# videosegmentation/video_segment

Measured on AMD Instinct MI355X. Metric: over-segmented frames/sec at 1080p, higher is better.
Workload: dtype f32

## Files before the change

### include/vsg.h

```cpp
#ifndef VSG_H_
#define VSG_H_

#include <stddef.h>
#include <stdint.h>

#ifdef __cplusplus
extern "C" {
#endif

#define VSG_OK 0
#define VSG_ERR_INVALID -1
#define VSG_ERR_DEVICE -2
#define VSG_ERR_STATE -3
#define VSG_ERR_INTERNAL -4

#define VSG_MEM_HOST 0
#define VSG_MEM_DEVICE 1

typedef struct vsg_stream vsg_stream;
typedef struct vsg_graph vsg_graph;

typedef struct vsg_options {
  int presmoothing;
  float frac_min_region_size;
// ... 215 lines not shown
                          const int32_t** nbr_csr_ptr, const int32_t** nbr_csr_idx);
int vsg_graph_get_intervals(vsg_graph* g, int frame, const vsg_interval** intervals, size_t* n);
int vsg_graph_smoothed(vsg_graph* g, int t, float* out );
int vsg_graph_spatial_buckets(vsg_graph* g, int t, uint16_t* out );
int vsg_graph_temporal_buckets(vsg_graph* g, int t, uint16_t* out , int32_t* prev_idx);
int vsg_graph_list_slots(vsg_graph* g, int list, uint32_t* slots_out, int32_t* offsets_out);
int vsg_graph_node_roots(vsg_graph* g, int32_t* out);
int vsg_graph_node_states(vsg_graph* g, int32_t* root, float* mean, int32_t* size, int32_t* constraint,
                          uint8_t* flags);
int vsg_graph_merge_stats(const vsg_graph* g, int64_t* forced_regular_small);
int vsg_graph_timings(const vsg_graph* g, vsg_timings* t);
int vsg_graph_diagnostics(const vsg_graph* g, vsg_diagnostics* d);
int vsg_graph_merge_paths(const vsg_graph* g, vsg_merge_paths* out);
int vsg_graph_spine_paths(const vsg_graph* g, vsg_spine_paths* out);

int vsg_debug_sort_pairs(const uint32_t* keys, const uint32_t* values, int n, int end_bit,
                         uint32_t* keys_out, uint32_t* values_out, int device);
int vsg_debug_sort_pairs_timed(const uint32_t* keys, const uint32_t* values, int n, int end_bit,
                               uint32_t* keys_out, uint32_t* values_out, int device, int impl, int reps,
                               double* avg_us);
int vsg_debug_exclusive_sum(const int32_t* in, int n, int32_t* out, int64_t* total);
int vsg_debug_runs_of_sorted_keys(const uint32_t* keys, int n, int32_t* seg_off, int32_t* seg_cnt,
                                  int32_t* num_runs);

#ifdef __cplusplus
}
#endif
#endif
```

### video_segment_amd/_lib.py

```python
import ctypes as C
import os
import subprocess

_HERE = os.path.dirname(os.path.abspath(__file__))
CSRC_DIR = os.path.join(_HERE, "csrc")
LIB_PATH = os.path.join(_HERE, "lib", "libvsg_hip.so")

VSG_OK = 0
VSG_ERR_INVALID, VSG_ERR_DEVICE, VSG_ERR_STATE, VSG_ERR_INTERNAL = -1, -2, -3, -4
VSG_MEM_HOST = 0
VSG_MEM_DEVICE = 1


class VsgOptions(C.Structure):
    _fields_ = [
        ("presmoothing", C.c_int),
        ("frac_min_region_size", C.c_float),
        ("chunk_size", C.c_int),
        ("chunk_overlap_ratio", C.c_float),
        ("num_constraint_frames", C.c_int),
        ("enforce_n4_connectivity", C.c_int),
        ("enforce_spatial_connectedness", C.c_int),
        ("color_distance", C.c_int),
        ("device", C.c_int),
# ... 117 lines not shown
    "vsg_stream_create", "vsg_stream_destroy", "vsg_stream_process_frame", "vsg_stream_chunk_size",
    "vsg_stream_result_bytes", "vsg_stream_result_id_image", "vsg_stream_last_merge_stats",
    "vsg_stream_keep_node_states", "vsg_stream_last_node_states",
    "vsg_stream_last_timings", "vsg_stream_last_diagnostics", "vsg_stream_last_merge_paths", "vsg_stream_last_spine_paths",
    "vsg_stream_last_boundary_paths",
    "vsg_stream_last_smoothed", "vsg_stream_export_halo",
    "vsg_stream_import_halo", "vsg_stream_expect_halo", "vsg_stream_restart",
    "vsg_chain_create", "vsg_chain_destroy", "vsg_chain_info", "vsg_chain_send_halo",
    "vsg_chain_recv_halo", "vsg_chain_exchange_halo",
    "vsg_regionseg_default_options", "vsg_regionseg_create", "vsg_regionseg_destroy", "vsg_regionseg_process_frame",
    "vsg_regionseg_result_bytes", "vsg_bgr_to_lab",
    "vsg_graph_create", "vsg_graph_destroy", "vsg_graph_add_frame_bgr",
    "vsg_graph_add_frame_features", "vsg_graph_add_virtual_frame", "vsg_graph_add_temporal",
    "vsg_graph_add_frame_features_temporal", "vsg_graph_list_slots",
    "vsg_graph_finish_building", "vsg_graph_segment_spatially", "vsg_graph_segment", "vsg_graph_obtain_results",
    "vsg_graph_num_frames", "vsg_graph_num_regions", "vsg_graph_num_neighbor_links",
    "vsg_graph_region_sizes", "vsg_graph_index_image", "vsg_graph_get_regions",
    "vsg_graph_get_intervals", "vsg_graph_smoothed",
    "vsg_graph_spatial_buckets", "vsg_graph_temporal_buckets", "vsg_graph_node_roots",
    "vsg_graph_node_states",
    "vsg_graph_merge_stats", "vsg_graph_timings", "vsg_graph_diagnostics", "vsg_graph_merge_paths",
    "vsg_graph_spine_paths",
    "vsg_debug_sort_pairs", "vsg_debug_sort_pairs_timed", "vsg_debug_exclusive_sum", "vsg_debug_runs_of_sorted_keys",
]


def build(force=False):
    subprocess.check_call(["make", "-C", CSRC_DIR, "-j8", "-s"])
    return LIB_PATH


_lib = None


def lib():
    global _lib
    if _lib is not None:
        return _lib
    if not os.path.exists(LIB_PATH):
        raise RuntimeError(
            "libvsg_hip.so is missing (%s): build the HIP extension first; there is no fallback "
            "path" % LIB_PATH)
    try:
        import torch
    except ImportError:
        pass
# ... 55 lines not shown
    L.vsg_graph_segment.argtypes = [vp, C.c_int, C.c_int]
    L.vsg_graph_obtain_results.argtypes = [vp, C.c_int, C.c_int, C.c_int]
    L.vsg_graph_num_frames.argtypes = [vp]
    L.vsg_graph_num_regions.argtypes = [vp]
    L.vsg_graph_num_neighbor_links.argtypes = [vp]
    L.vsg_graph_num_neighbor_links.restype = C.c_int64
    L.vsg_graph_region_sizes.argtypes = [vp, vp, vp]
    L.vsg_graph_index_image.argtypes = [vp, C.c_int, vp]
    L.vsg_graph_get_regions.argtypes = [vp, C.POINTER(vp), C.POINTER(C.c_size_t), C.POINTER(vp),
                                        C.POINTER(vp)]
    L.vsg_graph_get_intervals.argtypes = [vp, C.c_int, C.POINTER(vp), C.POINTER(C.c_size_t)]
    L.vsg_graph_smoothed.argtypes = [vp, C.c_int, vp]
    L.vsg_graph_spatial_buckets.argtypes = [vp, C.c_int, vp]
    L.vsg_graph_temporal_buckets.argtypes = [vp, C.c_int, vp, vp]
    L.vsg_graph_node_roots.argtypes = [vp, vp]
    L.vsg_graph_node_states.argtypes = [vp, vp, vp, vp, vp, vp]
    L.vsg_graph_merge_stats.argtypes = [vp, vp]
    L.vsg_graph_timings.argtypes = [vp, C.POINTER(VsgTimings)]
    L.vsg_graph_diagnostics.argtypes = [vp, C.POINTER(VsgDiagnostics)]
    L.vsg_graph_merge_paths.argtypes = [vp, C.POINTER(VsgMergePaths)]
    L.vsg_graph_spine_paths.argtypes = [vp, C.POINTER(VsgSpinePaths)]
    L.vsg_debug_exclusive_sum.argtypes = [vp, C.c_int, vp, C.POINTER(C.c_int64)]
    L.vsg_debug_runs_of_sorted_keys.argtypes = [vp, C.c_int, vp, vp, C.POINTER(C.c_int32)]
    _lib = L
    return L


class VsgError(RuntimeError):

    def __init__(self, msg, code=None):
        super().__init__(msg)
        self.code = code


def memory_stats(device=-1):
    st = VsgMemoryStats()
    check(lib().vsg_device_memory_stats(device, C.byref(st)))
    return st.as_dict()


def memory_trim(device=-1):
    check(lib().vsg_device_memory_trim(device))


def memory_limit(nbytes, device=-1):
    check(lib().vsg_device_memory_limit(device, int(nbytes)))
# ... 6 lines not shown
```

### video_segment_amd/csrc/capi.cpp

```cpp
#include <algorithm>
#include <cstring>
#include <memory>
#include <string>
#include <vector>

#include <rccl/rccl.h>

#include <chrono>
#include <cstdio>
#include <fstream>
#include <thread>

#include "../../include/vsg.h"
#include "region_segmentation.h"
#include "scan_device.h"
#include "stream.h"

namespace {

thread_local std::string g_last_error;

template <class F>
int Guard(F&& f) {
  try {
// ... 759 lines not shown
}

int vsg_debug_runs_of_sorted_keys(const uint32_t* keys, int n, int32_t* seg_off, int32_t* seg_cnt,
                                  int32_t* num_runs) {
  return Guard([&] {
    VSG_REQUIRE(keys && seg_off && seg_cnt && num_runs && n >= 0, VSG_ERR_INVALID, "bad argument");
    RequireDevice(-1);
    if (n == 0) return;
    vsg::DevBuf<uint32_t> d_keys((size_t)n);
    vsg::DevBuf<int32_t> d_off((size_t)n), d_cnt((size_t)n), sums(vsg::kScanMaxTiles), d_runs(1);
    DebugStream st;
    VSG_HIP(hipMemcpyAsync(d_keys.get(), keys, (size_t)n * 4, hipMemcpyHostToDevice, st.s));
    VSG_HIP(hipMemcpyAsync(d_off.get(), seg_off, (size_t)n * 4, hipMemcpyHostToDevice, st.s));
    VSG_HIP(hipMemcpyAsync(d_cnt.get(), seg_cnt, (size_t)n * 4, hipMemcpyHostToDevice, st.s));
    vsg::RunsOfSortedKeys(vsg::ScanScratch{sums.get(), nullptr}, d_keys.get(), n, d_off.get(), d_cnt.get(), d_runs.get(),
                          st.s);
    VSG_HIP(hipMemcpyAsync(seg_off, d_off.get(), (size_t)n * 4, hipMemcpyDeviceToHost, st.s));
    VSG_HIP(hipMemcpyAsync(seg_cnt, d_cnt.get(), (size_t)n * 4, hipMemcpyDeviceToHost, st.s));
    VSG_HIP(hipMemcpyAsync(num_runs, d_runs.get(), 4, hipMemcpyDeviceToHost, st.s));
    VSG_HIP(hipStreamSynchronize(st.s));
  });
}

int vsg_graph_create(int width, int height, int max_frames, int l1, int device, vsg_graph** out) {
  return Guard([&] {
    VSG_REQUIRE(out, VSG_ERR_INVALID, "null argument");
    RequireFrameSize(width, height);
    RequireDevice(device);
    std::unique_ptr<vsg_graph> g(new vsg_graph);
    g->device = ResolveDevice(device);
    DeviceGuard dg(g->device);
    g->W = width;
    g->H = height;
    g->wh = (size_t)width * height;
    VSG_HIP(hipStreamCreateWithFlags(&g->stream, hipStreamNonBlocking));
    g->g.reset(new vsg::DenseGraphHip(width, height, max_frames, l1 != 0, g->stream));
    g->pre.reset(new vsg::Preprocessor(width, height, g->stream));
    std::memset(&g->timings, 0, sizeof(g->timings));
    *out = g.release();
  });
}

void vsg_graph_destroy(vsg_graph* g) {
  if (!g) return;
  (void)Guard([&] {
    DeviceGuard dg(g->device);
// ... 388 lines not shown
```

### video_segment_amd/csrc/device_graph.h

```cpp
#ifndef VSG_DEVICE_GRAPH_H_
#define VSG_DEVICE_GRAPH_H_

#include <functional>

#include "common.h"

namespace vsg {

constexpr uint8_t kFlagFinalized = 1;
constexpr uint8_t kFlagNoDesc = 2;
constexpr uint8_t kFlagTentative = 4;
constexpr uint8_t kFlagHub = 8;
constexpr uint8_t kFlagHubBroken = 16;
constexpr uint8_t kFlagHubExcluded = 32;
constexpr int kHubExclCap = 16384;
constexpr int kHubMaxAttempts = 4;
constexpr int kHubMaxSplits = 64;
constexpr int kHubCutCap = 64;
constexpr int kHubListInts = 4 + kHubExclCap + 3 * kHubCutCap;

struct NodeArrays {
  int32_t* parent;
  float4* desc_sz;
  int32_t* cons;
// ... 40 lines not shown
  int32_t* chunk;
  int32_t* offsets;
  uint32_t* slots;
  int per_px;
};
constexpr int kEdgeSortMaxLists = 2;
void LaunchSpatialKeys(const float* feat, int W, int H, int l1, uint16_t* keys, int32_t* hist,
                       hipStream_t s);
void LaunchTemporalKeys(const float* cur, const float* prev, const float* flow, int W, int H,
                        int l1, int is_virtual, uint16_t* keys, int32_t* prev_idx, int32_t* hist,
                        hipStream_t s);
void LaunchBucketSort(const EdgeSortList* lists, int n_lists, size_t n_px, hipStream_t s);
void LaunchInitNodes(const float* feat, size_t n, int base, const int32_t* cons_in,
                     NodeArrays nodes, hipStream_t s);
void LaunchInitVirtualNodes(const int32_t* labels, size_t n, int base, int num_labels,
                            int32_t* first_scratch, NodeArrays nodes, hipStream_t s);

constexpr int kScanMaxTiles = 4096;
struct ScanScratch {
  int32_t* sums;
  hipStream_t owner = nullptr;
};

void DebugExclusiveSum(const ScanScratch& sc, const int32_t* in, int32_t* out, int n, int32_t* total, hipStream_t s);

size_t SortPairsU32HandTempBytes(int n);
void SortPairsU32Hand(void* temp, size_t temp_bytes, const uint32_t* keys_in, uint32_t* keys_out,
                      const uint32_t* vals_in, uint32_t* vals_out, int n, int end_bit, hipStream_t s);
size_t SortPairsU32LibTempBytes(int n);
void SortPairsU32Lib(void* temp, size_t temp_bytes, const uint32_t* keys_in, uint32_t* keys_out,
                     const uint32_t* vals_in, uint32_t* vals_out, int n, int end_bit, hipStream_t s);
size_t SortPairsU32TempBytes(int n);
void SortPairsU32(void* temp, size_t temp_bytes, const uint32_t* keys_in, uint32_t* keys_out,
                  const uint32_t* vals_in, uint32_t* vals_out, int n, int end_bit, hipStream_t s);
bool SortPairsU32TakesHand(int n);
size_t SortKeysU64TempBytes(int n);
void SortKeysU64(void* temp, size_t temp_bytes, const unsigned long long* in,
                 unsigned long long* out, int n,
                 hipStream_t s);
size_t UniqueU64TempBytes(int n);
void UniqueU64(void* temp, size_t temp_bytes, const unsigned long long* in,
               unsigned long long* out,
               int32_t* num_out, int n, hipStream_t s);

constexpr int kMailValues = 4;
struct MailSlot {
// ... 259 lines not shown
```

### video_segment_amd/csrc/merge_spine.hip

```cpp
#include <algorithm>
#include <chrono>
#include <cstdlib>
#include <cstdio>
#include <unordered_map>
#include <vector>

#include "merge_common.h"
#include "scan_device.h"

namespace vsg {

namespace {

constexpr int kNone = -1;

static inline unsigned Blocks(size_t n) { return (unsigned)((n + 255) / 256); }

__device__ __forceinline__ int CompOf(const int32_t* __restrict__ comp_base, int K, int e) {
  int lo = 0, hi = K;
  while (hi - lo > 1) {
    const int mid = (lo + hi) >> 1;
    if (comp_base[mid] <= e) lo = mid; else hi = mid;
  }
  return lo;
}

// ... 11 lines not shown
    const int lo = CompOf(comp_base, K, e);
    const int pos = comp_off[lo] + (e - comp_base[lo]);
    u = s_ra[pos];
    v = s_rb[pos];
    eu[e] = u;
    ev[e] = v;
    estate[e] = 0;
  }
  const int pu = __shfl_up(u, 1), pv = __shfl_up(v, 1);
  const bool first = (threadIdx.x & 63) == 0;
  if (valid && (first || (u != pu && u != pv))) {
    cc[u] = u;
    best[u] = 0xffffffffu;
  }
  if (valid && v != u && (first || (v != pu && v != pv))) {
    cc[v] = v;
    best[v] = 0xffffffffu;
  }
}

constexpr int kAliveSlots = 32;
__device__ __forceinline__ uint32_t BorKey(int round, int e) { return ((uint32_t)(31 - round) << 27) | (uint32_t)e; }

__global__ __launch_bounds__(256) void k_bor_min(int n, const int32_t* __restrict__ list,
                                                  const int32_t* __restrict__ list_len, int round,
                                                  const int32_t* __restrict__ eu,
                                                  const int32_t* __restrict__ ev, int32_t* __restrict__ estate,
                                                  int32_t* __restrict__ cc, uint32_t* __restrict__ best,
                                                  int32_t* __restrict__ ecu, int32_t* __restrict__ ecv,
                                                  int32_t* __restrict__ alive, const int32_t* __restrict__ gate,
                                                  int32_t* __restrict__ next_len) {
  if (blockIdx.x == 0 && threadIdx.x == 0) *next_len = 0;
  if (gate && *gate == 0) return;
  const int i = blockIdx.x * 256 + threadIdx.x;
  if (list_len) n = min(n, *list_len);
  const int e = i < n ? (list ? list[i] : i) : -1;
  bool live = false;
  int cu = -1, cv = -1;
  if (e >= 0 && round == 0) {
    cu = eu[e];
    cv = ev[e];
    live = true;
  } else if (e >= 0 && estate[e] == 0) {
    cu = CcFind(cc, eu[e]);
    cv = CcFind(cc, ev[e]);
    if (cu == cv) {
      estate[e] = 2;
      cu = cv = -1;
    } else {
      live = true;
      ecu[e] = cu;
      ecv[e] = cv;
    }
  }
  const int pu = __shfl_up(cu, 1), pv = __shfl_up(cv, 1), pe = __shfl_up(e, 1);
  if (live) {
    const uint32_t key = BorKey(round, e);
    const bool has_prev = (threadIdx.x & 63) != 0 && pe < e;
    if (!(has_prev && (cu == pu || cu == pv)) && key < best[cu]) atomicMin(&best[cu], key);
    if (!(has_prev && (cv == pu || cv == pv)) && key < best[cv]) atomicMin(&best[cv], key);
  }
  const int cnt = __syncthreads_count(live);
  if (cnt && threadIdx.x == 0) atomicAdd(&alive[(blockIdx.x % kAliveSlots) * 16], cnt);
}

__global__ __launch_bounds__(256) void k_bor_hook(int n, const int32_t* __restrict__ list,
                                                   const int32_t* __restrict__ list_len, int round,
                                                   const int32_t* __restrict__ eu, const int32_t* __restrict__ ev,
                                                   int32_t* __restrict__ estate, int32_t* __restrict__ cc,
                                                   const uint32_t* __restrict__ best,
                                                   const int32_t* __restrict__ ecu, const int32_t* __restrict__ ecv,
                                                   const int32_t* __restrict__ alive,
                                                   unsigned long long* __restrict__ mail, unsigned mail_seq,
                                                   const int32_t* __restrict__ gate, int32_t* __restrict__ total_out) {
  const int i = blockIdx.x * 256 + threadIdx.x;
  const bool idle = gate && *gate == 0;
  if (blockIdx.x == 0) {
    int v = (!idle && threadIdx.x < kAliveSlots) ? alive[threadIdx.x * 16] : 0;
    for (int off = 32; off > 0; off >>= 1) v += __shfl_down(v, off);
    if (threadIdx.x == 0) {
      *total_out = v;
      MailPost(mail, mail_seq, 0, v);
    }
  }
  if (idle) return;
  if (list_len) n = min(n, *list_len);
  if (i >= n) return;
  const int e = list ? list[i] : i;
  if (estate[e] != 0) return;
  const uint32_t key = BorKey(round, e);
  const int cu = round == 0 ? eu[e] : ecu[e], cv = round == 0 ? ev[e] : ecv[e];
  if (best[cu] == key || best[cv] == key) {
    CcUnion(cc, eu[e], ev[e]);
    estate[e] = 1;
  }
}

constexpr int kBorCompactPer = 8;
__global__ __launch_bounds__(256) void k_bor_compact(int n, const int32_t* __restrict__ list,
                                                      const int32_t* __restrict__ list_len,
                                                      const int32_t* __restrict__ estate, int32_t* __restrict__ out,
                                                      int32_t* __restrict__ out_len) {
  __shared__ int wave_tot[4];
  __shared__ int block_base;
  if (list_len) n = min(n, *list_len);
  const int lane = threadIdx.x & 63, w = threadIdx.x >> 6;
  int e[kBorCompactPer];
  unsigned long long m[kBorCompactPer];
  int mine = 0;
#pragma unroll
  for (int k = 0; k < kBorCompactPer; ++k) {
    const int i = (blockIdx.x * kBorCompactPer + k) * 256 + threadIdx.x;
    e[k] = i < n ? (list ? list[i] : i) : -1;
    const bool keep = e[k] >= 0 && estate[e[k]] == 0;
    m[k] = __ballot(keep);
    mine += (int)__popcll(m[k]);
  }
  if (lane == 0) wave_tot[w] = mine;
  __syncthreads();
  if (threadIdx.x == 0) {
    const int total = wave_tot[0] + wave_tot[1] + wave_tot[2] + wave_tot[3];
    block_base = total ? atomicAdd(out_len, total) : 0;
  }
  __syncthreads();
  int at = block_base;
  for (int q = 0; q < w; ++q) at += wave_tot[q];
#pragma unroll
  for (int k = 0; k < kBorCompactPer; ++k) {
    if ((m[k] >> lane) & 1ull) out[at + (int)__popcll(m[k] & ((1ull << lane) - 1ull))] = e[k];
    at += (int)__popcll(m[k]);
  }
}

constexpr int kRootStride = 16;
__global__ __launch_bounds__(256) void k_spine_pick_root(int mE, int K, const int32_t* __restrict__ eu,
                                                          const int32_t* __restrict__ ev,
                                                          const int32_t* __restrict__ comp_base, NodeArrays nodes,
                                                          unsigned long long* __restrict__ root_key) {
  __shared__ unsigned long long red[256];
  __shared__ int comp0;
  const int i = blockIdx.x * 256 + threadIdx.x;
  const int e = i < K ? comp_base[i] : (i - K) * kRootStride;
  unsigned long long key = 0;
  int k = -1;
  if (e < mE) {
    k = CompOf(comp_base, K, e);
    const int u = eu[e], v = ev[e];
    const unsigned su = (unsigned)__float_as_int(nodes.desc_sz[u].w);
    const unsigned sv = (unsigned)__float_as_int(nodes.desc_sz[v].w);
    const unsigned long long ku = ((unsigned long long)su << 32) | (unsigned)(~u);
    const unsigned long long kv = ((unsigned long long)sv << 32) | (unsigned)(~v);
    key = ku > kv ? ku : kv;
  }
// ... 951 lines not shown
    out[2 * i] = seg_off[seg];
    out[2 * i + 1] = cnt;
  }
}

struct Pool {
  int32_t* base;
  size_t cap, used = 0;
  bool ok = true;
  size_t mark() const { return used; }
  void release(size_t m) { used = m; }
  int32_t* take(size_t n) {
    n = (n + 63) & ~(size_t)63;
    if (used + n > cap) {
      ok = false;
      return base;
    }
    int32_t* p = base + used;
    used += n;
    return p;
  }
};

}

size_t SpinePoolInts(size_t max_edges) { return 16 * max_edges + 64 * 1024; }

int SelectLargeSegments(int max_segs, const int32_t* num_segs, const int32_t* seg_off, const int32_t* seg_cnt,
                        int min_cnt, long long max_edges, MergeScratch& S, hipStream_t s, SpineInput* out,
                        long long* wanted_edges) {
  out->segs.clear();
  if (wanted_edges) *wanted_edges = 0;
  Mailbox& mb = *S.mail;
  VSG_REQUIRE(mb.list_cap >= 2 * kSpineListCap, -4, "mailbox list too small");
  std::vector<int32_t> large(1 + 2 * kSpineListCap);
  int found = 0;
  for (;; min_cnt *= 4) {
    int32_t* d_found = TakeZeroed(S, 1);
    hipLaunchKernelGGL(k_list_large_segments, dim3(Blocks(max_segs)), dim3(256), 0, s, max_segs, num_segs, seg_off,
                       seg_cnt, min_cnt, d_found, mb.list_dev);
    const MailSlot m = NextMail(mb);
    LaunchMailPost(m, d_found, nullptr, nullptr, nullptr, s);
    MailWait(m, 1, &found, s);
    if (found <= kSpineListCap) break;
  }
  large[0] = found;
// ... 16 lines not shown
    all += sizes[(size_t)i];
  }
  if (wanted_edges) *wanted_edges = all;
  std::sort(sizes.begin(), sizes.end(), std::greater<int>());
  long long sum = 0;
  int taken = 0, thr = 0x7fffffff;
  for (int i = 0; i < found && i < 256;) {
    int j = i;
    long long group = 0;
    while (j < found && sizes[(size_t)j] == sizes[(size_t)i]) group += sizes[(size_t)j++];
    if (sum + group > max_edges || j > 256) break;
    sum += group;
    taken = j;
    thr = sizes[(size_t)i];
    i = j;
  }
  if (taken == 0) return 0x7fffffff;
  for (int i = 0; i < found; ++i) {
    if (large[2 + 2 * i] >= thr) out->segs.push_back(SpineSeg{large[1 + 2 * i], large[2 + 2 * i]});
  }
  return thr;
}

bool RunSpineComponents(const SpineInput& in, const WorkerArgs& wa, MergeScratch& S, hipStream_t s,
                        const SpineWorkers& run_workers, size_t pool_used, int depth) {
  const int K = (int)in.segs.size();
  if (K == 0) return false;
  std::vector<int32_t> base(K + 1, 0), off(K);
  for (int k = 0; k < K; ++k) {
    base[k + 1] = base[k] + in.segs[k].cnt;
    off[k] = in.segs[k].off;
  }
  const int mE = base[K];
  VSG_REQUIRE(mE < (1 << 27), -4, "spine: too many edges for the stamped ranks");
  double tph[8] = {0};
  auto Mark = [&](int i) {
    if (!S.spine_debug) return;
    VSG_HIP(hipStreamSynchronize(s));
    tph[i] = std::chrono::duration<double, std::milli>(std::chrono::steady_clock::now().time_since_epoch()).count();
  };
  Mark(0);
  SpinePaths& sp = S.sp;
  if (pool_used >= S.spine_pool_ints) {
    ++sp.pool_fallbacks[0];
    return false;
  }
  ++sp.replays;
  sp.components += K;
  if (depth >= 1) ++sp.nested_replays;
  sp.deepest_level = std::max<int64_t>(sp.deepest_level, depth);
  Pool pool{S.spine_pool + pool_used, S.spine_pool_ints - pool_used};
  int32_t* d_base = pool.take(K + 1);
  int32_t* d_off = pool.take(K);
  int32_t* root_vertex = pool.take(K);
  int32_t* comp_spine = pool.take(K + 1);
  unsigned long long* root_key = reinterpret_cast<unsigned long long*>(TakeZeroed(S, 2 * (size_t)K));
  int32_t* scalars = pool.take(64);
  int32_t* eu = pool.take(mE);
  int32_t* ev = pool.take(mE);
  int32_t* estate = pool.take(mE);
  int32_t* flag = pool.take(mE);
  int32_t* scan = pool.take(mE);
  int32_t* side_key = pool.take(mE);
  int32_t* spine_flag = pool.take(mE);
  if (!pool.ok) {
    ++sp.pool_fallbacks[1];
    return false;
  }
  int32_t* cc = S.cc;
  uint32_t* best = reinterpret_cast<uint32_t*>(S.nmap[0]);
  int32_t* firstq = S.nmap[1];
  int32_t* childidx = S.nmap[2];

  VSG_REQUIRE(d_off == d_base + (((size_t)K + 1 + 63) & ~(size_t)63), -4, "spine: off does not follow base in the pool");
  const size_t off_at = (size_t)(d_off - d_base);
  if (int32_t* src = TakeStageRing(S, off_at + K)) {
    std::copy(base.begin(), base.end(), src);
    std::fill(src + K + 1, src + off_at, 0);
    std::copy(off.begin(), off.end(), src + off_at);
    VSG_HIP(hipMemcpyAsync(d_base, src, (off_at + K) * sizeof(int32_t), hipMemcpyHostToDevice, s));
  } else {
    VSG_HIP(hipMemcpyAsync(d_base, base.data(), (K + 1) * sizeof(int32_t), hipMemcpyHostToDevice, s));
    VSG_HIP(hipMemcpyAsync(d_off, off.data(), K * sizeof(int32_t), hipMemcpyHostToDevice, s));
  }
  hipLaunchKernelGGL(k_spine_gather, dim3(Blocks(mE)), dim3(256), 0, s, mE, K, d_base, d_off, wa.s_ra,
                     wa.s_rb, eu, ev, estate, cc, best);
  hipLaunchKernelGGL(k_spine_pick_root, dim3(Blocks((size_t)K + (mE + kRootStride - 1) / kRootStride)), dim3(256), 0,
                     s, mE, K, eu, ev, d_base, wa.nodes, root_key);
  hipLaunchKernelGGL(k_spine_roots, dim3((K + 63) / 64), dim3(64), 0, s, K, root_key, root_vertex, childidx);

  int dbg_rounds = 0;
  auto NowMs = [] {
    return std::chrono::duration<double, std::milli>(std::chrono::steady_clock::now().time_since_epoch()).count();
  };
  const bool dbg_big = S.spine_debug && mE > (8 << 20);
  if (dbg_big) {
    VSG_HIP(hipStreamSynchronize(s));
    std::fprintf(stderr, "[vsg]   forest: gather+root %.2f ms\n", NowMs() - tph[0]);
  }
  {
    const size_t forest_mark = pool.mark();
    const int32_t* list = nullptr;
    const int32_t* list_len = nullptr;
    int n_list = mE;
    int32_t* lists[2] = {nullptr, nullptr};
    int which = 0;
    const int ahead_max = getenv("VSG_BOR_AHEAD") ? atoi(getenv("VSG_BOR_AHEAD")) : (4 << 20);
    const int compact_min = getenv("VSG_BOR_COMPACT_MIN") ? atoi(getenv("VSG_BOR_COMPACT_MIN")) : (1 << 16);
    MailSlot waiting[2];
    int n_waiting = 0;
    const int32_t* gate = nullptr;
    int32_t* len_words = scalars + 8;
    int32_t* gate_words = scalars + 12;
    int len_cur = 0;
    for (int round = 0;; ++round) {
      dbg_rounds = round;
      VSG_REQUIRE(round < 32, -4, "spine: the spanning forest did not converge");
      ++sp.forest_rounds;
      int32_t* d_ctr = TakeZeroed(S, 16 * kAliveSlots + 4);
      int32_t* d_next_len = len_words + (len_cur ^ 1);
      hipLaunchKernelGGL(k_bor_min, dim3(Blocks(n_list)), dim3(256), 0, s, n_list, list, list_len, round, eu, ev,
                         estate, cc, best, side_key, spine_flag, d_ctr, gate, d_next_len);
      const MailSlot m_alive = NextMail(*S.mail);
      hipLaunchKernelGGL(k_bor_hook, dim3(Blocks(n_list)), dim3(256), 0, s, n_list, list, list_len, round, eu, ev,
                         estate, cc, best, side_key, spine_flag, d_ctr, m_alive.dev, m_alive.seq, gate,
                         gate_words + (round & 1));
      gate = gate_words + (round & 1);
      waiting[n_waiting++] = m_alive;
      const int depth = n_list <= ahead_max ? 1 : 0;
      if (depth == 1) ++sp.forest_rounds_ahead;
      const double tr0 = dbg_big ? NowMs() : 0;
      int alive = -1;
      bool complete = false;
      while (n_waiting > depth) {
        MailWait(waiting[0], 1, &alive, s);
        waiting[0] = waiting[1];
        --n_waiting;
        if (alive == 0) {
          complete = true;
          break;
        }
      }
      if (dbg_big) std::fprintf(stderr, "[vsg]   forest round %d: %d in list, %d alive, %.2f ms\n", round, n_list, alive, NowMs() - tr0);
      if (complete) break;
      const bool compact = depth == 1 ? (round >= 1 && n_list > compact_min)
                                      : (alive < n_list / 2 && n_list > compact_min);
      if (!compact) continue;
      if (!lists[0]) {
        const size_t m = pool.mark();
        const size_t cap = depth == 1 ? (size_t)n_list : (size_t)alive;
        lists[0] = pool.take(cap);
        lists[1] = pool.take(cap);
        if (!pool.ok) {
          ++sp.forest_lists_refused;
          pool.ok = true;
          pool.release(m);
          lists[0] = lists[1] = nullptr;
        }
      }
      if (!lists[0]) continue;
      ++(depth == 1 ? sp.forest_compactions_ahead : sp.forest_compactions_sync);
      hipLaunchKernelGGL(k_bor_compact, dim3(Blocks(((size_t)n_list + kBorCompactPer - 1) / kBorCompactPer)),
                         dim3(256), 0, s, n_list, list, list_len, estate, lists[which], d_next_len);
      list = lists[which];
      list_len = d_next_len;
      len_cur ^= 1;
      which ^= 1;
      if (alive >= 0) n_list = std::min(n_list, alive);
    }
    pool.release(forest_mark);
  }
  Mark(1);
  const MailSlot m_mt = NextMail(*S.mail);
  FusedScan(S.scan, StateFlagValue{estate, 1}, FlagScanEmit{flag, scan}, TotalPostFinish{scalars + 1, m_mt.dev, m_mt.seq},
            mE, s);
  int mt = 0;
  MailWait(m_mt, 1, &mt, s);
  VSG_REQUIRE(mt > 0, -4, "spine: a component without tree edges");
  const int na = 2 * mt;
  int32_t* te_e = pool.take(mt);
  int32_t* child = pool.take(mt);
  int32_t* par = pool.take(mt);
  int32_t* jump[2] = {pool.take(mt), pool.take(mt)};
  int32_t* val[2] = {pool.take(mt), pool.take(mt)};
  int32_t* head = pool.take(mt);
  int32_t* sp_child = pool.take(mt);
  int32_t* sp_is_a = pool.take(mt);
  const size_t arcs_mark = pool.mark();

  uint32_t* ak_in = reinterpret_cast<uint32_t*>(pool.take(na));
  uint32_t* av_in = reinterpret_cast<uint32_t*>(pool.take(na));
  uint32_t* ak = reinterpret_cast<uint32_t*>(pool.take(na));
  uint32_t* av = reinterpret_cast<uint32_t*>(pool.take(na));
  int32_t* pos_arc = pool.take(na);
// ... 255 lines not shown
```

Before: 218.8.

## Restructure Boruvka spanning forest with compacted edge records carrying component roots

Moves the Boruvka spanning-forest loop into a reusable RunSpanningForest routine. After the first rounds it fuses the min-finding and compaction steps into one kernel that writes compacted records (edge id plus current component endpoints), so later rounds read contiguous lists instead of indirecting through estate, eu and ev. Union-find lookups are batched across several edges per thread, and hooking unions the cached component roots directly. This aims to cut memory traffic and launches per round, at the cost of extra pool memory for three-array lists and more complex kernels. It also adds a debug C API entry point for exercising the forest on its own.

```diff
diff --git a/include/vsg.h b/include/vsg.h
--- a/include/vsg.h
+++ b/include/vsg.h
@@ -261,6 +261,9 @@
 int vsg_debug_exclusive_sum(const int32_t* in, int n, int32_t* out, int64_t* total);
 int vsg_debug_runs_of_sorted_keys(const uint32_t* keys, int n, int32_t* seg_off, int32_t* seg_cnt,
                                   int32_t* num_runs);
+int vsg_debug_spanning_forest(const int32_t* eu, const int32_t* ev, int n_edges, int n_vertices,
+                              const int32_t* comp_base, int n_comps, int ahead, int compact_min, int wide_min,
+                              int64_t list_pool_ints, int32_t* estate, int64_t* counts);
 
 #ifdef __cplusplus
 }
diff --git a/video_segment_amd/_lib.py b/video_segment_amd/_lib.py
--- a/video_segment_amd/_lib.py
+++ b/video_segment_amd/_lib.py
@@ -163,6 +163,7 @@
     "vsg_graph_merge_stats", "vsg_graph_timings", "vsg_graph_diagnostics", "vsg_graph_merge_paths",
     "vsg_graph_spine_paths",
     "vsg_debug_sort_pairs", "vsg_debug_sort_pairs_timed", "vsg_debug_exclusive_sum", "vsg_debug_runs_of_sorted_keys",
+    "vsg_debug_spanning_forest",
 ]
 
 
@@ -264,6 +265,8 @@
     L.vsg_graph_spine_paths.argtypes = [vp, C.POINTER(VsgSpinePaths)]
     L.vsg_debug_exclusive_sum.argtypes = [vp, C.c_int, vp, C.POINTER(C.c_int64)]
     L.vsg_debug_runs_of_sorted_keys.argtypes = [vp, C.c_int, vp, vp, C.POINTER(C.c_int32)]
+    L.vsg_debug_spanning_forest.argtypes = [vp, vp, C.c_int, C.c_int, vp, C.c_int, C.c_int, C.c_int, C.c_int,
+                                            C.c_int64, vp, vp]
     _lib = L
     return L
 
diff --git a/video_segment_amd/csrc/capi.cpp b/video_segment_amd/csrc/capi.cpp
--- a/video_segment_amd/csrc/capi.cpp
+++ b/video_segment_amd/csrc/capi.cpp
@@ -805,6 +805,27 @@
   });
 }
 
+int vsg_debug_spanning_forest(const int32_t* eu, const int32_t* ev, int n_edges, int n_vertices,
+                              const int32_t* comp_base, int n_comps, int ahead, int compact_min, int wide_min,
+                              int64_t list_pool_ints, int32_t* estate, int64_t* counts) {
+  return Guard([&] {
+    VSG_REQUIRE(eu && ev && comp_base && estate && counts && n_edges >= 1 && n_edges < (1 << 27) && n_vertices >= 2 &&
+                    n_comps >= 1 && n_comps <= n_edges && list_pool_ints >= 0,
+                VSG_ERR_INVALID, "bad argument");
+    VSG_REQUIRE(comp_base[0] == 0 && comp_base[n_comps] == n_edges, VSG_ERR_INVALID, "bad component bases");
+    for (int k = 0; k < n_comps; ++k) {
+      VSG_REQUIRE(comp_base[k] < comp_base[k + 1], VSG_ERR_INVALID, "bad component bases");
+    }
+    for (int e = 0; e < n_edges; ++e) {
+      VSG_REQUIRE(eu[e] >= 0 && eu[e] < n_vertices && ev[e] >= 0 && ev[e] < n_vertices && eu[e] != ev[e],
+                  VSG_ERR_INVALID, "bad edge end");
+    }
+    RequireDevice(-1);
+    vsg::DebugSpanningForest(eu, ev, n_edges, n_vertices, comp_base, n_comps, ahead, compact_min, wide_min, list_pool_ints, estate,
+                             counts);
+  });
+}
+
 int vsg_graph_create(int width, int height, int max_frames, int l1, int device, vsg_graph** out) {
   return Guard([&] {
     VSG_REQUIRE(out, VSG_ERR_INVALID, "null argument");
diff --git a/video_segment_amd/csrc/device_graph.h b/video_segment_amd/csrc/device_graph.h
--- a/video_segment_amd/csrc/device_graph.h
+++ b/video_segment_amd/csrc/device_graph.h
@@ -86,6 +86,9 @@
   hipStream_t owner = nullptr;
 };
 
+void DebugSpanningForest(const int32_t* eu, const int32_t* ev, int n_edges, int n_vertices, const int32_t* comp_base,
+                         int n_comps, int ahead, int compact_min, int wide_min, long long list_pool_ints,
+                         int32_t* estate, int64_t* counts);
 void DebugExclusiveSum(const ScanScratch& sc, const int32_t* in, int32_t* out, int n, int32_t* total, hipStream_t s);
 
 size_t SortPairsU32HandTempBytes(int n);
diff --git a/video_segment_amd/csrc/merge_spine.hip b/video_segment_amd/csrc/merge_spine.hip
--- a/video_segment_amd/csrc/merge_spine.hip
+++ b/video_segment_amd/csrc/merge_spine.hip
@@ -2,6 +2,7 @@
 #include <chrono>
 #include <cstdlib>
 #include <cstdio>
+#include <cstring>
 #include <unordered_map>
 #include <vector>
 
@@ -59,9 +60,7 @@
 constexpr int kAliveSlots = 32;
 __device__ __forceinline__ uint32_t BorKey(int round, int e) { return ((uint32_t)(31 - round) << 27) | (uint32_t)e; }
 
-__global__ __launch_bounds__(256) void k_bor_min(int n, const int32_t* __restrict__ list,
-                                                  const int32_t* __restrict__ list_len, int round,
-                                                  const int32_t* __restrict__ eu,
+__global__ __launch_bounds__(256) void k_bor_min(int n, int round, const int32_t* __restrict__ eu,
                                                   const int32_t* __restrict__ ev, int32_t* __restrict__ estate,
                                                   int32_t* __restrict__ cc, uint32_t* __restrict__ best,
                                                   int32_t* __restrict__ ecu, int32_t* __restrict__ ecv,
@@ -70,8 +69,7 @@
   if (blockIdx.x == 0 && threadIdx.x == 0) *next_len = 0;
   if (gate && *gate == 0) return;
   const int i = blockIdx.x * 256 + threadIdx.x;
-  if (list_len) n = min(n, *list_len);
-  const int e = i < n ? (list ? list[i] : i) : -1;
+  const int e = i < n ? i : -1;
   bool live = false;
   int cu = -1, cv = -1;
   if (e >= 0 && round == 0) {
@@ -79,8 +77,8 @@
     cv = ev[e];
     live = true;
   } else if (e >= 0 && estate[e] == 0) {
-    cu = CcFind(cc, eu[e]);
-    cv = CcFind(cc, ev[e]);
+    cu = CcFind(cc, round >= 2 ? ecu[e] : eu[e]);
+    cv = CcFind(cc, round >= 2 ? ecv[e] : ev[e]);
     if (cu == cv) {
       estate[e] = 2;
       cu = cv = -1;
@@ -90,10 +88,10 @@
       ecv[e] = cv;
     }
   }
-  const int pu = __shfl_up(cu, 1), pv = __shfl_up(cv, 1), pe = __shfl_up(e, 1);
+  const int pu = __shfl_up(cu, 1), pv = __shfl_up(cv, 1);
   if (live) {
     const uint32_t key = BorKey(round, e);
-    const bool has_prev = (threadIdx.x & 63) != 0 && pe < e;
+    const bool has_prev = (threadIdx.x & 63) != 0;
     if (!(has_prev && (cu == pu || cu == pv)) && key < best[cu]) atomicMin(&best[cu], key);
     if (!(has_prev && (cv == pu || cv == pv)) && key < best[cv]) atomicMin(&best[cv], key);
   }
@@ -101,56 +99,123 @@
   if (cnt && threadIdx.x == 0) atomicAdd(&alive[(blockIdx.x % kAliveSlots) * 16], cnt);
 }
 
-__global__ __launch_bounds__(256) void k_bor_hook(int n, const int32_t* __restrict__ list,
-                                                   const int32_t* __restrict__ list_len, int round,
-                                                   const int32_t* __restrict__ eu, const int32_t* __restrict__ ev,
-                                                   int32_t* __restrict__ estate, int32_t* __restrict__ cc,
-                                                   const uint32_t* __restrict__ best,
+__device__ __forceinline__ void BorReportAlive(bool idle, const int32_t* __restrict__ alive,
+                                               unsigned long long* __restrict__ mail, unsigned mail_seq,
+                                               int32_t* __restrict__ total_out) {
+  int v = (!idle && threadIdx.x < kAliveSlots) ? alive[threadIdx.x * 16] : 0;
+  for (int off = 32; off > 0; off >>= 1) v += __shfl_down(v, off);
+  if (threadIdx.x == 0) {
+    *total_out = v;
+    MailPost(mail, mail_seq, 0, v);
+  }
+}
+
+__global__ __launch_bounds__(256) void k_bor_hook(int n, int round, const int32_t* __restrict__ eu,
+                                                   const int32_t* __restrict__ ev, int32_t* __restrict__ estate,
+                                                   int32_t* __restrict__ cc, const uint32_t* __restrict__ best,
                                                    const int32_t* __restrict__ ecu, const int32_t* __restrict__ ecv,
                                                    const int32_t* __restrict__ alive,
                                                    unsigned long long* __restrict__ mail, unsigned mail_seq,
                                                    const int32_t* __restrict__ gate, int32_t* __restrict__ total_out) {
-  const int i = blockIdx.x * 256 + threadIdx.x;
+  const int e = blockIdx.x * 256 + threadIdx.x;
   const bool idle = gate && *gate == 0;
-  if (blockIdx.x == 0) {
-    int v = (!idle && threadIdx.x < kAliveSlots) ? alive[threadIdx.x * 16] : 0;
-    for (int off = 32; off > 0; off >>= 1) v += __shfl_down(v, off);
-    if (threadIdx.x == 0) {
-      *total_out = v;
-      MailPost(mail, mail_seq, 0, v);
-    }
-  }
-  if (idle) return;
-  if (list_len) n = min(n, *list_len);
-  if (i >= n) return;
-  const int e = list ? list[i] : i;
-  if (estate[e] != 0) return;
+  if (blockIdx.x == 0 && threadIdx.x < 64) BorReportAlive(idle, alive, mail, mail_seq, total_out);
+  if (idle || e >= n) return;
+  if (round != 0 && estate[e] != 0) return;
   const uint32_t key = BorKey(round, e);
   const int cu = round == 0 ? eu[e] : ecu[e], cv = round == 0 ? ev[e] : ecv[e];
   if (best[cu] == key || best[cv] == key) {
-    CcUnion(cc, eu[e], ev[e]);
+    CcUnion(cc, cu, cv);
     estate[e] = 1;
   }
 }
 
-constexpr int kBorCompactPer = 8;
-__global__ __launch_bounds__(256) void k_bor_compact(int n, const int32_t* __restrict__ list,
-                                                      const int32_t* __restrict__ list_len,
-                                                      const int32_t* __restrict__ estate, int32_t* __restrict__ out,
-                                                      int32_t* __restrict__ out_len) {
+constexpr int kBorTreeBit = 1 << 30;
+constexpr int kBorPer = 8;
+struct BorList {
+  int32_t* e;
+  int32_t* cu;
+  int32_t* cv;
+};
+
+template <int N>
+__device__ __forceinline__ void CcFindMany(int32_t* cc, int (&x)[N]) {
+  int p[N];
+#pragma unroll
+  for (int j = 0; j < N; ++j) p[j] = x[j] >= 0 ? cc[x[j]] : x[j];
+  for (;;) {
+    bool more = false;
+#pragma unroll
+    for (int j = 0; j < N; ++j) more |= p[j] != x[j];
+    if (!more) break;
+    int q[N];
+#pragma unroll
+    for (int j = 0; j < N; ++j) q[j] = p[j] != x[j] ? cc[p[j]] : p[j];
+#pragma unroll
+    for (int j = 0; j < N; ++j) {
+      if (p[j] != x[j]) {
+        if (q[j] != p[j]) cc[x[j]] = q[j];
+        x[j] = p[j];
+        p[j] = q[j];
+      }
+    }
+  }
+}
+
+template <int kPer>
+__global__ __launch_bounds__(256) void k_bor_min_rec(int n, BorList in, const int32_t* __restrict__ in_len, int round,
+                                                      const int32_t* __restrict__ eu, const int32_t* __restrict__ ev,
+                                                      const int32_t* __restrict__ estate, int32_t* __restrict__ cc,
+                                                      uint32_t* __restrict__ best, BorList out,
+                                                      int32_t* __restrict__ out_len, int32_t* __restrict__ alive,
+                                                      const int32_t* __restrict__ gate, int32_t* __restrict__ zero_len) {
   __shared__ int wave_tot[4];
   __shared__ int block_base;
-  if (list_len) n = min(n, *list_len);
+  if (blockIdx.x == 0 && threadIdx.x == 0) *zero_len = 0;
+  if (gate && *gate == 0) return;
+  if (in_len) n = min(n, *in_len);
   const int lane = threadIdx.x & 63, w = threadIdx.x >> 6;
-  int e[kBorCompactPer];
-  unsigned long long m[kBorCompactPer];
+  int e[kPer], r[2 * kPer];
+  unsigned long long m[kPer];
   int mine = 0;
 #pragma unroll
-  for (int k = 0; k < kBorCompactPer; ++k) {
-    const int i = (blockIdx.x * kBorCompactPer + k) * 256 + threadIdx.x;
-    e[k] = i < n ? (list ? list[i] : i) : -1;
-    const bool keep = e[k] >= 0 && estate[e[k]] == 0;
-    m[k] = __ballot(keep);
+  for (int k = 0; k < kPer; ++k) {
+    const int i = (blockIdx.x * kPer + k) * 256 + threadIdx.x;
+    int ee = -1, a = -1, b = -1;
+    if (i < n) {
+      if (in.e) {
+        ee = in.e[i];
+        if (ee & kBorTreeBit) {
+          ee = -1;
+        } else {
+          a = in.cu[i];
+          b = in.cv[i];
+        }
+      } else if (estate[i] == 0) {
+        ee = i;
+        a = eu[i];
+        b = ev[i];
+      }
+    }
+    e[k] = ee;
+    r[2 * k] = a;
+    r[2 * k + 1] = b;
+  }
+  CcFindMany<2 * kPer>(cc, r);
+#pragma unroll
+  for (int k = 0; k < kPer; ++k) {
+    const int ee = e[k];
+    const bool live = ee >= 0 && r[2 * k] != r[2 * k + 1];
+    if (!live) r[2 * k] = r[2 * k + 1] = -1;
+    const int a = r[2 * k], b = r[2 * k + 1];
+    const int pu = __shfl_up(a, 1), pv = __shfl_up(b, 1), pe = __shfl_up(ee, 1);
+    if (live) {
+      const uint32_t key = BorKey(round, ee);
+      const bool has_prev = lane != 0 && pe < ee;
+      if (!(has_prev && (a == pu || a == pv)) && key < best[a]) atomicMin(&best[a], key);
+      if (!(has_prev && (b == pu || b == pv)) && key < best[b]) atomicMin(&best[b], key);
+    }
+    m[k] = __ballot(live);
     mine += (int)__popcll(m[k]);
   }
   if (lane == 0) wave_tot[w] = mine;
@@ -158,14 +223,43 @@
   if (threadIdx.x == 0) {
     const int total = wave_tot[0] + wave_tot[1] + wave_tot[2] + wave_tot[3];
     block_base = total ? atomicAdd(out_len, total) : 0;
+    if (total) atomicAdd(&alive[(blockIdx.x % kAliveSlots) * 16], total);
   }
   __syncthreads();
   int at = block_base;
   for (int q = 0; q < w; ++q) at += wave_tot[q];
 #pragma unroll
-  for (int k = 0; k < kBorCompactPer; ++k) {
-    if ((m[k] >> lane) & 1ull) out[at + (int)__popcll(m[k] & ((1ull << lane) - 1ull))] = e[k];
+  for (int k = 0; k < kPer; ++k) {
+    if ((m[k] >> lane) & 1ull) {
+      const int o = at + (int)__popcll(m[k] & ((1ull << lane) - 1ull));
+      out.e[o] = e[k];
+      out.cu[o] = r[2 * k];
+      out.cv[o] = r[2 * k + 1];
+    }
     at += (int)__popcll(m[k]);
+  }
+}
+
+__global__ __launch_bounds__(256) void k_bor_hook_rec(int n, BorList list, const int32_t* __restrict__ list_len,
+                                                       int round, int32_t* __restrict__ estate,
+                                                       int32_t* __restrict__ cc, const uint32_t* __restrict__ best,
+                                                       const int32_t* __restrict__ alive,
+                                                       unsigned long long* __restrict__ mail, unsigned mail_seq,
+                                                       const int32_t* __restrict__ gate,
+                                                       int32_t* __restrict__ total_out) {
+  const int i = blockIdx.x * 256 + threadIdx.x;
+  const bool idle = gate && *gate == 0;
+  if (blockIdx.x == 0 && threadIdx.x < 64) BorReportAlive(idle, alive, mail, mail_seq, total_out);
+  if (idle) return;
+  n = min(n, *list_len);
+  if (i >= n) return;
+  const int e = list.e[i];
+  const uint32_t key = BorKey(round, e);
+  const int cu = list.cu[i], cv = list.cv[i];
+  if (best[cu] == key || best[cv] == key) {
+    CcUnion(cc, cu, cv);
+    estate[e] = 1;
+    list.e[i] = e | kBorTreeBit;
   }
 }
 
@@ -1163,6 +1257,116 @@
   }
 };
 
+struct ForestEdges {
+  int mE, K;
+  const int32_t* base;
+  const int32_t* off;
+  const int32_t* ra;
+  const int32_t* rb;
+};
+struct ForestScratch {
+  int32_t* eu;
+  int32_t* ev;
+  int32_t* ecu;
+  int32_t* ecv;
+  int32_t* cc;
+  uint32_t* best;
+  int32_t* scalars;
+};
+struct ForestKnobs {
+  int ahead_max = 4 << 20;
+  int compact_min = 1 << 16;
+  int wide_min = 4 << 20;
+};
+
+int RunSpanningForest(const ForestEdges& E, const ForestScratch& F, int32_t* estate, const ForestKnobs& knobs,
+                      Pool& pool, MergeScratch& S, hipStream_t s) {
+  const int mE = E.mE;
+  VSG_REQUIRE(mE < (1 << 27), -4, "spine: too many edges for the stamped ranks");
+  SpinePaths& sp = S.sp;
+  auto NowMs = [] {
+    return std::chrono::duration<double, std::milli>(std::chrono::steady_clock::now().time_since_epoch()).count();
+  };
+  const bool dbg_big = S.spine_debug && mE > (8 << 20);
+  hipLaunchKernelGGL(k_spine_gather, dim3(Blocks(mE)), dim3(256), 0, s, mE, E.K, E.base, E.off, E.ra, E.rb, F.eu, F.ev,
+                     estate, F.cc, F.best);
+  const size_t forest_mark = pool.mark();
+  int n_list = mE;
+  BorList lists[2] = {{nullptr, nullptr, nullptr}, {nullptr, nullptr, nullptr}};
+  bool rec = false;
+  bool have_list = false;
+  MailSlot waiting[2];
+  int n_waiting = 0;
+  const int32_t* gate = nullptr;
+  int32_t* len_words = F.scalars;
+  int32_t* gate_words = F.scalars + 4;
+  int round = 0;
+  for (;; ++round) {
+    VSG_REQUIRE(round < 32, -4, "spine: the spanning forest did not converge");
+    ++sp.forest_rounds;
+    const int depth = n_list <= knobs.ahead_max ? 1 : 0;
+    if (!rec && round >= 1 && n_list > knobs.compact_min) {
+      const size_t m = pool.mark();
+      const size_t cap = (size_t)n_list;
+      lists[0] = BorList{pool.take(cap), F.ecu, F.ecv};
+      lists[1] = BorList{pool.take(cap), pool.take(cap), pool.take(cap)};
+      if (pool.ok) {
+        rec = true;
+      } else {
+        ++sp.forest_lists_refused;
+        pool.ok = true;
+        pool.release(m);
+      }
+    }
+    int32_t* d_ctr = TakeZeroed(S, 16 * kAliveSlots + 4);
+    int32_t* d_zero_len = len_words + (round + 1) % 3;
+    const MailSlot m_alive = NextMail(*S.mail);
+    if (rec) {
+      ++(depth == 1 ? sp.forest_compactions_ahead : sp.forest_compactions_sync);
+      const BorList in = have_list ? lists[(round & 1) ^ 1] : BorList{nullptr, nullptr, nullptr};
+      const BorList out = lists[round & 1];
+      int32_t* d_out_len = len_words + round % 3;
+      const int32_t* d_in_len = have_list ? len_words + (round + 2) % 3 : nullptr;
+      if (n_list >= knobs.wide_min) {
+        hipLaunchKernelGGL(k_bor_min_rec<kBorPer>, dim3(Blocks(((size_t)n_list + kBorPer - 1) / kBorPer)), dim3(256), 0,
+                           s, n_list, in, d_in_len, round, F.eu, F.ev, estate, F.cc, F.best, out, d_out_len, d_ctr, gate,
+                           d_zero_len);
+      } else {
+        hipLaunchKernelGGL(k_bor_min_rec<1>, dim3(Blocks(n_list)), dim3(256), 0, s, n_list, in, d_in_len, round, F.eu,
+                           F.ev, estate, F.cc, F.best, out, d_out_len, d_ctr, gate, d_zero_len);
+      }
+      hipLaunchKernelGGL(k_bor_hook_rec, dim3(Blocks(n_list)), dim3(256), 0, s, n_list, out, d_out_len, round, estate,
+                         F.cc, F.best, d_ctr, m_alive.dev, m_alive.seq, gate, gate_words + (round & 1));
+      have_list = true;
+    } else {
+      hipLaunchKernelGGL(k_bor_min, dim3(Blocks(n_list)), dim3(256), 0, s, n_list, round, F.eu, F.ev, estate, F.cc,
+                         F.best, F.ecu, F.ecv, d_ctr, gate, d_zero_len);
+      hipLaunchKernelGGL(k_bor_hook, dim3(Blocks(n_list)), dim3(256), 0, s, n_list, round, F.eu, F.ev, estate, F.cc,
+                         F.best, F.ecu, F.ecv, d_ctr, m_alive.dev, m_alive.seq, gate, gate_words + (round & 1));
+    }
+    gate = gate_words + (round & 1);
+    waiting[n_waiting++] = m_alive;
+    if (depth == 1) ++sp.forest_rounds_ahead;
+    const double tr0 = dbg_big ? NowMs() : 0;
+    int alive = -1;
+    bool complete = false;
+    while (n_waiting > depth) {
+      MailWait(waiting[0], 1, &alive, s);
+      waiting[0] = waiting[1];
+      --n_waiting;
+      if (alive == 0) {
+        complete = true;
+        break;
+      }
+    }
+    if (dbg_big) std::fprintf(stderr, "[vsg]   forest round %d: %d in list, %d alive, %.2f ms\n", round, n_list, alive, NowMs() - tr0);
+    if (complete) break;
+    if (have_list && alive >= 0) n_list = std::min(n_list, alive);
+  }
+  pool.release(forest_mark);
+  return round;
+}
+
 }
 
 size_t SpinePoolInts(size_t max_edges) { return 16 * max_edges + 64 * 1024; }
@@ -1225,6 +1429,63 @@
   return thr;
 }
 
+void DebugSpanningForest(const int32_t* eu, const int32_t* ev, int n_edges, int n_vertices, const int32_t* comp_base,
+                         int n_comps, int ahead, int compact_min, int wide_min, long long list_pool_ints,
+                         int32_t* estate, int64_t* counts) {
+  const size_t mE = (size_t)n_edges, K = (size_t)n_comps, nv = (size_t)n_vertices;
+  struct Owner {
+    hipStream_t s = nullptr;
+    void* mail = nullptr;
+    ~Owner() {
+      if (s) (void)hipStreamDestroy(s);
+      if (mail) CacheFree(mail);
+    }
+  } own;
+  VSG_HIP(hipStreamCreateWithFlags(&own.s, hipStreamNonBlocking));
+  hipStream_t s = own.s;
+  DevBuf<int32_t> d_ra(mE), d_rb(mE), d_base(K + 1), d_eu(mE), d_ev(mE), d_ecu(mE), d_ecv(mE), d_estate(mE), d_cc(nv),
+      d_best(nv), d_scalars(64), d_zero(kZeroArenaInts + 2 * 4096), d_pool((size_t)std::max(list_pool_ints, 64ll));
+  Mailbox mail;
+  const int slots = 16;
+  const size_t mail_bytes = (size_t)slots * kMailValues * sizeof(unsigned long long);
+  own.mail = CacheAlloc(mail_bytes, kCacheMappedCoherent);
+  std::memset(own.mail, 0, mail_bytes);
+  void* mail_dev = nullptr;
+  VSG_HIP(hipHostGetDevicePointer(&mail_dev, own.mail, 0));
+  mail.host = static_cast<volatile unsigned long long*>(own.mail);
+  mail.dev = static_cast<unsigned long long*>(mail_dev);
+  mail.slots = slots;
+  mail.seq = 0;
+  ZeroPool zeros;
+  zeros.base = d_zero.get();
+  zeros.cap = d_zero.size();
+  MergeScratch S{};
+  S.mail = &mail;
+  S.zeros = &zeros;
+  S.main_stream = s;
+  VSG_HIP(hipMemsetAsync(d_zero.get(), 0, d_zero.size() * sizeof(int32_t), s));
+  VSG_HIP(hipMemcpyAsync(d_ra.get(), eu, mE * 4, hipMemcpyHostToDevice, s));
+  VSG_HIP(hipMemcpyAsync(d_rb.get(), ev, mE * 4, hipMemcpyHostToDevice, s));
+  VSG_HIP(hipMemcpyAsync(d_base.get(), comp_base, (K + 1) * 4, hipMemcpyHostToDevice, s));
+  LaunchInitIdentity(d_cc.get(), nv, s);
+  Pool pool{d_pool.get(), list_pool_ints > 0 ? (size_t)list_pool_ints : 0};
+  ForestKnobs knobs;
+  knobs.ahead_max = ahead;
+  knobs.compact_min = compact_min;
+  knobs.wide_min = wide_min;
+  RunSpanningForest(ForestEdges{n_edges, n_comps, d_base.get(), d_base.get(), d_ra.get(), d_rb.get()},
+                    ForestScratch{d_eu.get(), d_ev.get(), d_ecu.get(), d_ecv.get(), d_cc.get(),
+                                  reinterpret_cast<uint32_t*>(d_best.get()), d_scalars.get()},
+                    d_estate.get(), knobs, pool, S, s);
+  VSG_HIP(hipMemcpyAsync(estate, d_estate.get(), mE * 4, hipMemcpyDeviceToHost, s));
+  VSG_HIP(hipStreamSynchronize(s));
+  counts[0] = S.sp.forest_rounds;
+  counts[1] = S.sp.forest_rounds_ahead;
+  counts[2] = S.sp.forest_compactions_ahead;
+  counts[3] = S.sp.forest_compactions_sync;
+  counts[4] = S.sp.forest_lists_refused;
+}
+
 bool RunSpineComponents(const SpineInput& in, const WorkerArgs& wa, MergeScratch& S, hipStream_t s,
                         const SpineWorkers& run_workers, size_t pool_used, int depth) {
   const int K = (int)in.segs.size();
@@ -1257,7 +1518,6 @@
   int32_t* d_off = pool.take(K);
   int32_t* root_vertex = pool.take(K);
   int32_t* comp_spine = pool.take(K + 1);
-  unsigned long long* root_key = reinterpret_cast<unsigned long long*>(TakeZeroed(S, 2 * (size_t)K));
   int32_t* scalars = pool.take(64);
   int32_t* eu = pool.take(mE);
   int32_t* ev = pool.take(mE);
@@ -1286,93 +1546,17 @@
     VSG_HIP(hipMemcpyAsync(d_base, base.data(), (K + 1) * sizeof(int32_t), hipMemcpyHostToDevice, s));
     VSG_HIP(hipMemcpyAsync(d_off, off.data(), K * sizeof(int32_t), hipMemcpyHostToDevice, s));
   }
-  hipLaunchKernelGGL(k_spine_gather, dim3(Blocks(mE)), dim3(256), 0, s, mE, K, d_base, d_off, wa.s_ra,
-                     wa.s_rb, eu, ev, estate, cc, best);
+  ForestKnobs knobs;
+  knobs.ahead_max = getenv("VSG_BOR_AHEAD") ? atoi(getenv("VSG_BOR_AHEAD")) : knobs.ahead_max;
+  knobs.compact_min = getenv("VSG_BOR_COMPACT_MIN") ? atoi(getenv("VSG_BOR_COMPACT_MIN")) : knobs.compact_min;
+  knobs.wide_min = getenv("VSG_BOR_WIDE_MIN") ? atoi(getenv("VSG_BOR_WIDE_MIN")) : knobs.wide_min;
+  const int dbg_rounds = RunSpanningForest(ForestEdges{mE, K, d_base, d_off, wa.s_ra, wa.s_rb},
+                                           ForestScratch{eu, ev, side_key, spine_flag, cc, best, scalars + 8}, estate,
+                                           knobs, pool, S, s);
+  unsigned long long* root_key = reinterpret_cast<unsigned long long*>(TakeZeroed(S, 2 * (size_t)K));
   hipLaunchKernelGGL(k_spine_pick_root, dim3(Blocks((size_t)K + (mE + kRootStride - 1) / kRootStride)), dim3(256), 0,
                      s, mE, K, eu, ev, d_base, wa.nodes, root_key);
   hipLaunchKernelGGL(k_spine_roots, dim3((K + 63) / 64), dim3(64), 0, s, K, root_key, root_vertex, childidx);
-
-  int dbg_rounds = 0;
-  auto NowMs = [] {
-    return std::chrono::duration<double, std::milli>(std::chrono::steady_clock::now().time_since_epoch()).count();
-  };
-  const bool dbg_big = S.spine_debug && mE > (8 << 20);
-  if (dbg_big) {
-    VSG_HIP(hipStreamSynchronize(s));
-    std::fprintf(stderr, "[vsg]   forest: gather+root %.2f ms\n", NowMs() - tph[0]);
-  }
-  {
-    const size_t forest_mark = pool.mark();
-    const int32_t* list = nullptr;
-    const int32_t* list_len = nullptr;
-    int n_list = mE;
-    int32_t* lists[2] = {nullptr, nullptr};
-    int which = 0;
-    const int ahead_max = getenv("VSG_BOR_AHEAD") ? atoi(getenv("VSG_BOR_AHEAD")) : (4 << 20);
-    const int compact_min = getenv("VSG_BOR_COMPACT_MIN") ? atoi(getenv("VSG_BOR_COMPACT_MIN")) : (1 << 16);
-    MailSlot waiting[2];
-    int n_waiting = 0;
-    const int32_t* gate = nullptr;
-    int32_t* len_words = scalars + 8;
-    int32_t* gate_words = scalars + 12;
-    int len_cur = 0;
-    for (int round = 0;; ++round) {
-      dbg_rounds = round;
-      VSG_REQUIRE(round < 32, -4, "spine: the spanning forest did not converge");
-      ++sp.forest_rounds;
-      int32_t* d_ctr = TakeZeroed(S, 16 * kAliveSlots + 4);
-      int32_t* d_next_len = len_words + (len_cur ^ 1);
-      hipLaunchKernelGGL(k_bor_min, dim3(Blocks(n_list)), dim3(256), 0, s, n_list, list, list_len, round, eu, ev,
-                         estate, cc, best, side_key, spine_flag, d_ctr, gate, d_next_len);
-      const MailSlot m_alive = NextMail(*S.mail);
-      hipLaunchKernelGGL(k_bor_hook, dim3(Blocks(n_list)), dim3(256), 0, s, n_list, list, list_len, round, eu, ev,
-                         estate, cc, best, side_key, spine_flag, d_ctr, m_alive.dev, m_alive.seq, gate,
-                         gate_words + (round & 1));
-      gate = gate_words + (round & 1);
-      waiting[n_waiting++] = m_alive;
-      const int depth = n_list <= ahead_max ? 1 : 0;
-      if (depth == 1) ++sp.forest_rounds_ahead;
-      const double tr0 = dbg_big ? NowMs() : 0;
-      int alive = -1;
-      bool complete = false;
-      while (n_waiting > depth) {
-        MailWait(waiting[0], 1, &alive, s);
-        waiting[0] = waiting[1];
-        --n_waiting;
-        if (alive == 0) {
-          complete = true;
-          break;
-        }
-      }
-      if (dbg_big) std::fprintf(stderr, "[vsg]   forest round %d: %d in list, %d alive, %.2f ms\n", round, n_list, alive, NowMs() - tr0);
-      if (complete) break;
-      const bool compact = depth == 1 ? (round >= 1 && n_list > compact_min)
-                                      : (alive < n_list / 2 && n_list > compact_min);
-      if (!compact) continue;
-      if (!lists[0]) {
-        const size_t m = pool.mark();
-        const size_t cap = depth == 1 ? (size_t)n_list : (size_t)alive;
-        lists[0] = pool.take(cap);
-        lists[1] = pool.take(cap);
-        if (!pool.ok) {
-          ++sp.forest_lists_refused;
-          pool.ok = true;
-          pool.release(m);
-          lists[0] = lists[1] = nullptr;
-        }
-      }
-      if (!lists[0]) continue;
-      ++(depth == 1 ? sp.forest_compactions_ahead : sp.forest_compactions_sync);
-      hipLaunchKernelGGL(k_bor_compact, dim3(Blocks(((size_t)n_list + kBorCompactPer - 1) / kBorCompactPer)),
-                         dim3(256), 0, s, n_list, list, list_len, estate, lists[which], d_next_len);
-      list = lists[which];
-      list_len = d_next_len;
-      len_cur ^= 1;
-      which ^= 1;
-      if (alive >= 0) n_list = std::min(n_list, alive);
-    }
-    pool.release(forest_mark);
-  }
   Mark(1);
   const MailSlot m_mt = NextMail(*S.mail);
   FusedScan(S.scan, StateFlagValue{estate, 1}, FlagScanEmit{flag, scan}, TotalPostFinish{scalars + 1, m_mt.dev, m_mt.seq},
```

After: 218.7. About the same (-0.0%).
